# xxlong0/NeuralUDF

Measured on NVIDIA H100. Metric: ray-samples/sec (render_core fwd+bwd), higher is better.
Workload: dtype f32

## Files before the change

### neuraludf_b200/csrc/gemm_simt.cuh

```cuda
#pragma once
#include "common.cuh"

namespace nudf {

constexpr int GS_BM = 128, GS_BN = 128, GS_BK = 8, GS_PAD = 4, GS_THREADS = 256;

__device__ __forceinline__ unsigned long long pack2(float x, float y) {
  unsigned long long r;
  asm("mov.b64 %0, {%1, %2};" : "=l"(r) : "f"(x), "f"(y));
  return r;
}
__device__ __forceinline__ void unpack2(unsigned long long v, float& x, float& y) {
  asm("mov.b64 {%0, %1}, %2;" : "=f"(x), "=f"(y) : "l"(v));
}
__device__ __forceinline__ void ffma2(unsigned long long& d, unsigned long long a, unsigned long long b) {
  float dx, dy, ax, ay, bx, by;
  unpack2(d, dx, dy);
  unpack2(a, ax, ay);
  unpack2(b, bx, by);
  d = pack2(fmaf(ax, bx, dx), fmaf(ay, by, dy));
}

template <bool KC>
__device__ __forceinline__ float4 gs_fetch(const float* __restrict__ src, int64_t ld, int64_t mn0, int64_t mn_total, int k0,
// ... 125 lines not shown

__device__ __forceinline__ void ld4(const float* __restrict__ base, int64_t ld, int64_t row, int col, int nv, float out[4]) {
  const float* p = base + row * ld + col;
  if (nv == 4 && ((ld & 3) == 0) && ((col & 3) == 0) && aligned16(base)) {
    float4 t = *reinterpret_cast<const float4*>(p);
    out[0] = t.x; out[1] = t.y; out[2] = t.z; out[3] = t.w;
  } else {
#pragma unroll
    for (int j = 0; j < 4; ++j) out[j] = j < nv ? p[j] : 0.f;
  }
}
__device__ __forceinline__ void st4(float* __restrict__ base, int64_t ld, int64_t row, int col, int nv, const float v[4]) {
  float* p = base + row * ld + col;
  if (nv == 4 && ((ld & 3) == 0) && ((col & 3) == 0) && aligned16(base)) {
    *reinterpret_cast<float4*>(p) = make_float4(v[0], v[1], v[2], v[3]);
  } else {
#pragma unroll
    for (int j = 0; j < 4; ++j)
      if (j < nv) p[j] = v[j];
  }
}

#define NUDF_EPI_CALL                                                                                     \
  __device__ __forceinline__ void operator()(int64_t row, int col, const float acc[4], int nv) const {    \
    Aux aux;                                                                                              \
    load(row, col, nv, aux);                                                                              \
    apply(row, col, acc, nv, aux);                                                                        \
  }

struct EpiAct {
  float* C; int64_t ldc; const float* bias; int act; float post_scale;
  struct Aux { float b[4]; };
  __device__ __forceinline__ void load(int64_t, int col, int nv, Aux& x) const {
#pragma unroll
    for (int j = 0; j < 4; ++j) x.b[j] = (bias != nullptr && j < nv) ? bias[col + j] : 0.f;
  }
  __device__ __forceinline__ void apply(int64_t row, int col, const float acc[4], int nv, const Aux& x) const {
    float v[4];
#pragma unroll
    for (int j = 0; j < 4; ++j) {
      float t = acc[j] + x.b[j];
      if (act == ACT_RELU) t = fmaxf(t, 0.f);
      else if (act == ACT_SOFTPLUS100) t = softplus100(t);
      else if (act == ACT_SIGMOID) t = sigmoidf_(t);
      v[j] = t * post_scale;
    }
    st4(C, ldc, row, col, nv, v);
  }
  NUDF_EPI_CALL
};

struct EpiAtomicAdd {
  float* C; int64_t ldc;
  struct Aux {};
  __device__ __forceinline__ void load(int64_t, int, int, Aux&) const {}
  __device__ __forceinline__ void apply(int64_t row, int col, const float acc[4], int nv, const Aux&) const {
    float* p = C + row * ldc + col;
    if (nv == 4 && ((ldc & 3) == 0) && ((col & 3) == 0) && aligned16(C)) {
      asm volatile("red.global.add.v4.f32 [%0], {%1, %2, %3, %4};" ::"l"(p), "f"(acc[0]), "f"(acc[1]), "f"(acc[2]), "f"(acc[3])
                   : "memory");
      return;
    }
#pragma unroll
    for (int j = 0; j < 4; ++j)
      if (j < nv) atomicAdd(p + j, acc[j]);
  }
  NUDF_EPI_CALL
};


struct EpiSplitStore {
  float* ws; int64_t slice; int64_t ld;
  struct Aux {};
  __device__ __forceinline__ void load(int64_t, int, int, Aux&) const {}
  __device__ __forceinline__ void apply(int64_t row, int col, const float acc[4], int nv, const Aux&) const {
    float* p = ws + blockIdx.z * slice + row * ld + col;
#pragma unroll
    for (int j = 0; j < 4; ++j)
      if (j < nv) p[j] = acc[j];
  }
  NUDF_EPI_CALL
};

template <class Epi>
__global__ void splitk_reduce_kernel(const float* __restrict__ ws, int64_t slice, int splits, int64_t M, int N, Epi epi) {
  const int ncq = (N + 3) / 4;
  const int64_t idx = (int64_t)blockIdx.x * blockDim.x + threadIdx.x;
  const int64_t row = idx / ncq;
  if (row >= M) return;
  const int col = (int)(idx - row * ncq) * 4;
  const int nv = N - col < 4 ? N - col : 4;
  float x[4] = {0.f, 0.f, 0.f, 0.f};
  for (int z = 0; z < splits; ++z) {
    const float* p = ws + z * slice + row * N + col;
#pragma unroll
    for (int j = 0; j < 4; ++j)
      if (j < nv) x[j] += p[j];
  }
  epi(row, col, x, nv);
}
static __global__ void vec_reduce_kernel(const float* __restrict__ ws, int splits, int64_t n, float* __restrict__ out) {
  const int64_t i = (int64_t)blockIdx.x * blockDim.x + threadIdx.x;
  if (i >= n) return;
  float t = 0.f;
  for (int z = 0; z < splits; ++z) t += ws[z * n + i];
  out[i] += t;
}
template <class Epi>
static inline int splitk_reduce(const float* ws, int splits, int64_t M, int N, const Epi& epi, cudaStream_t st) {
  const int64_t n = M * ((N + 3) / 4);
  splitk_reduce_kernel<Epi><<<(unsigned)cdiv(n, 256), 256, 0, st>>>(ws, M * N, splits, M, N, epi);
  NUDF_LAUNCH_OK();
  return 0;
}
static inline int vec_reduce(const float* ws, int splits, int64_t n, float* out, cudaStream_t st) {
  vec_reduce_kernel<<<(unsigned)cdiv(n, 256), 256, 0, st>>>(ws, splits, n, out);
  NUDF_LAUNCH_OK();
  return 0;
}
static inline int ws_splits(int want, int64_t per_split) {
  const int64_t cap = SPLIT_WS_FLOATS / (per_split > 0 ? per_split : 1);
  return (int)(want < cap ? want : (cap < 1 ? 1 : cap));
}

struct EpiRev {
  int n_main; float post_scale;
  const float* Anext; int64_t lda; float a_unscale;
  float* Dprev; int64_t ldd;
  float* Gpe; int64_t ldg;
  struct Aux { float a[4]; };
  __device__ __forceinline__ void load(int64_t row, int col, int nv, Aux& x) const {
    int n = n_main - col;
    n = n < nv ? n : nv;
    if (n > 0) ld4(Anext, lda, row, col, n, x.a);
    else { x.a[0] = x.a[1] = x.a[2] = x.a[3] = 0.f; }
  }
  __device__ __forceinline__ void apply(int64_t row, int col, const float acc[4], int nv, const Aux& x) const {
    if (col + nv <= n_main) {
      float d[4];
#pragma unroll
      for (int j = 0; j < 4; ++j) d[j] = acc[j] * post_scale * sig_from_softplus(x.a[j] * a_unscale);
      st4(Dprev, ldd, row, col, nv, d);
      return;
    }
#pragma unroll
    for (int j = 0; j < 4; ++j) {
      if (j >= nv) break;
      int c = col + j;
      float g = acc[j] * post_scale;
      if (c < n_main) Dprev[row * ldd + c] = g * sig_from_softplus(x.a[j] * a_unscale);
      else if (Gpe != nullptr) Gpe[row * ldg + (c - n_main)] = g;
    }
  }
  NUDF_EPI_CALL
};

struct EpiRevFinal {
  float* Ge; int64_t ldge; const float* Gpe; int64_t ldg;
  struct Aux { float g[4]; };
  __device__ __forceinline__ void load(int64_t row, int col, int nv, Aux& x) const {
    if (Gpe != nullptr) ld4(Gpe, ldg, row, col, nv, x.g);
    else { x.g[0] = x.g[1] = x.g[2] = x.g[3] = 0.f; }
  }
  __device__ __forceinline__ void apply(int64_t row, int col, const float acc[4], int nv, const Aux& x) const {
    float v[4];
#pragma unroll
    for (int j = 0; j < 4; ++j) v[j] = acc[j] + x.g[j];
    st4(Ge, ldge, row, col, nv, v);
  }
  NUDF_EPI_CALL
};

struct EpiTan {
  const float* Anext; int64_t lda; float a_unscale;
  const float* D; int64_t ldd;
  float* Q; int64_t ldq;
  float* AdotNext; int64_t ldn; float post_scale;
  struct Aux { float a[4], d[4]; };
  __device__ __forceinline__ void load(int64_t row, int col, int nv, Aux& x) const {
    ld4(Anext, lda, row, col, nv, x.a);
    ld4(D, ldd, row, col, nv, x.d);
  }
  __device__ __forceinline__ void apply(int64_t row, int col, const float acc[4], int nv, const Aux& x) const {
    float q[4], n[4];
#pragma unroll
    for (int j = 0; j < 4; ++j) {
      float s = sig_from_softplus(x.a[j] * a_unscale);
      q[j] = acc[j] * x.d[j] * (100.0f * (1.0f - s));
      n[j] = s * acc[j] * post_scale;
    }
    st4(Q, ldq, row, col, nv, q);
    st4(AdotNext, ldn, row, col, nv, n);
  }
  NUDF_EPI_CALL
};

struct EpiBwd {
  int n_main; float post_scale;
  const float* Anext; int64_t lda; float a_unscale;
// ... 105 lines not shown
```

### neuraludf_b200/csrc/gemm_tc.cuh

```cuda
#pragma once
#include <cuda.h>
#include <cudaTypedefs.h>
#include <cuda_bf16.h>

#include "gemm_simt.cuh"

namespace nudf {
namespace tc {

constexpr int BM = 128;
constexpr int BN = 128;
constexpr int BK = 64;
constexpr int THREADS = 256;
constexpr int A_HALF_BYTES = BM * BK * 2;
__host__ __device__ constexpr int b_plane_bytes(int wn) { return wn * BK * 2; }
__host__ __device__ constexpr int acc_ld(int wn) { return wn + 4; }

__host__ __device__ inline int pad16(int n) { return (n + 15) & ~15; }
__host__ __device__ inline int pad64(int k) { return (k + 63) & ~63; }

__host__ __device__ inline uint32_t sw128(uint32_t row, uint32_t k) {
  return (row >> 3) * 1024u + (row & 7u) * 128u + ((((k >> 3) ^ (row & 7u)) & 7u) << 4) + ((k & 7u) << 1);
}

constexpr int TN_PS = 32;
constexpr int TN_RING = 4;
constexpr uint32_t TN_F32_OPND = TN_PS * BM * 4;
constexpr uint32_t TN_F32_STAGE = 2 * TN_F32_OPND;
constexpr uint32_t TN_PLANE = BM * TN_PS * 2;
constexpr uint32_t TN_PLANE_STAGE = 4 * TN_PLANE;
struct TnMaps { CUtensorMap a, b; };
__host__ __device__ inline uint32_t sw128_mn(uint32_t mn, uint32_t k) {
  return (mn >> 6) * 4096u + (k >> 3) * 1024u + (k & 7u) * 128u + ((((mn >> 3) ^ k) & 7u) << 4) + ((mn & 7u) << 1);
}

constexpr uint32_t W_SLOT = BM * BK * 4;
static_assert(W_SLOT == 2 * A_HALF_BYTES, "a slot holds exactly the two bf16 planes of its slice");
__host__ __device__ constexpr int w_ring(int wn) { return wn == 256 ? 3 : 4; }

__device__ __forceinline__ uint32_t pack_bf16(float a, float b) {
  __nv_bfloat162 v = __floats2bfloat162_rn(a, b);
  return *reinterpret_cast<uint32_t*>(&v);
}
template <int NP>
__device__ __forceinline__ void split4(const float x[4], uint2 planes[NP]) {
  float r[4] = {x[0], x[1], x[2], x[3]};
#pragma unroll
  for (int p = 0; p < NP; ++p) {
    const uint32_t a = pack_bf16(r[0], r[1]), b = pack_bf16(r[2], r[3]);
    planes[p] = make_uint2(a, b);
    r[0] -= __uint_as_float(a << 16);
    r[1] -= __uint_as_float(a & 0xffff0000u);
    r[2] -= __uint_as_float(b << 16);
    r[3] -= __uint_as_float(b & 0xffff0000u);
  }
}
__host__ __device__ inline int nt_of(int np) { return np == 2 ? 256 : 128; }
__host__ __device__ inline int n_tiles(int N, int np) { return (N + nt_of(np) - 1) / nt_of(np); }
__host__ __device__ inline int tile_rows(int N, int t, int np) { int r = N - nt_of(np) * t; return pad16(r < nt_of(np) ? r : nt_of(np)); }
__host__ __device__ inline int64_t tile_elems(int N, int K, int t, int np) { return (int64_t)(pad64(K) / 64) * np * tile_rows(N, t, np) * 64; }
__host__ __device__ inline int64_t tile_offset(int N, int K, int t, int np) {
  int64_t o = 0;
  for (int i = 0; i < t; ++i) o += tile_elems(N, K, i, np);
  return o;
}
__host__ __device__ inline int64_t image_elems(int N, int K, int np) { return tile_offset(N, K, n_tiles(N, np), np); }

static __device__ __forceinline__ void tc_prep_weights_body(const float* __restrict__ W, int64_t ldw, int N, int K, int transposed, int np,
                                                            uint16_t* __restrict__ img, int64_t start, int64_t stride) {
  const int Kp = pad64(K);
  const int nt = n_tiles(N, np);
  int64_t total = 0;
  for (int t = 0; t < nt; ++t) total += (int64_t)tile_rows(N, t, np) * Kp;
  for (int64_t idx = start; idx < total; idx += stride) {
    int64_t rem = idx;
    int t = 0;
    while (rem >= (int64_t)tile_rows(N, t, np) * Kp) { rem -= (int64_t)tile_rows(N, t, np) * Kp; ++t; }
    const int rows = tile_rows(N, t, np);
    const int nl = (int)(rem / Kp), k = (int)(rem - (int64_t)nl * Kp);
    const int n = t * nt_of(np) + nl;
    float x = 0.f;
    if (n < N && k < K) x = transposed ? W[(int64_t)k * ldw + n] : W[(int64_t)n * ldw + k];
    const int s = k >> 6, kl = k & 63;
    uint16_t* base = img + tile_offset(N, K, t, np) + (int64_t)s * np * rows * 64;
    const uint32_t off = sw128((uint32_t)nl, (uint32_t)kl) >> 1;
    float r = x;
    for (int p = 0; p < np; ++p) {
      __nv_bfloat16 h = __float2bfloat16_rn(r);
      base[(int64_t)p * rows * 64 + off] = __bfloat16_as_ushort(h);
      r -= __bfloat162float(h);
    }
  }
}
static __global__ void tc_prep_weights_kernel(const float* __restrict__ W, int64_t ldw, int N, int K, int transposed, int np,
                                              uint16_t* __restrict__ img) {
  tc_prep_weights_body(W, ldw, N, K, transposed, np, img, (int64_t)blockIdx.x * blockDim.x + threadIdx.x, (int64_t)gridDim.x * blockDim.x);
}


__device__ __forceinline__ uint32_t smem_u32(const void* p) { return (uint32_t)__cvta_generic_to_shared(p); }
__device__ __forceinline__ uint8_t* align1024(uint8_t* p) {
  return reinterpret_cast<uint8_t*>((reinterpret_cast<uintptr_t>(p) + 1023) & ~(uintptr_t)1023);
}

__device__ __forceinline__ void mbar_init(uint64_t* bar, uint32_t count) {
  asm volatile("mbarrier.init.shared::cta.b64 [%0], %1;" ::"r"(smem_u32(bar)), "r"(count) : "memory");
}
__device__ __forceinline__ void mbar_arrive(uint64_t* bar) {
  asm volatile("mbarrier.arrive.shared::cta.b64 _, [%0];" ::"r"(smem_u32(bar)) : "memory");
}
__device__ __forceinline__ void mbar_arrive_expect_tx(uint64_t* bar, uint32_t bytes) {
  asm volatile("mbarrier.arrive.expect_tx.shared::cta.b64 _, [%0], %1;" ::"r"(smem_u32(bar)), "r"(bytes) : "memory");
}
__device__ __forceinline__ uint32_t mbar_try_wait(uint32_t addr, uint32_t parity) {
  uint32_t ok;
  asm volatile(
      "{\n"
      ".reg .pred p;\n"
      "mbarrier.try_wait.parity.shared::cta.b64 p, [%1], %2;\n"
      "selp.u32 %0, 1, 0, p;\n"
      "}\n"
      : "=r"(ok)
      : "r"(addr), "r"(parity)
      : "memory");
  return ok;
}
__device__ __forceinline__ void mbar_wait(uint64_t* bar, uint32_t parity) {
  const uint32_t addr = smem_u32(bar);
  while (!mbar_try_wait(addr, parity)) {
  }
}
__device__ __forceinline__ void fence_barrier_init() { asm volatile("fence.mbarrier_init.release.cluster;" ::: "memory"); }
__device__ __forceinline__ void fence_proxy_async() { asm volatile("fence.proxy.async.shared::cta;" ::: "memory"); }

__device__ __forceinline__ void bulk_g2s(void* smem_dst, const void* gmem_src, uint32_t bytes, uint64_t* bar) {
  asm volatile("cp.async.bulk.shared::cluster.global.mbarrier::complete_tx::bytes [%0], [%1], %2, [%3];" ::"r"(smem_u32(smem_dst)),
               "l"(gmem_src), "r"(bytes), "r"(smem_u32(bar))
               : "memory");
}

__device__ __forceinline__ void tma_load_2d(void* smem_dst, const CUtensorMap* map, int c, int k, uint64_t* bar) {
  asm volatile("cp.async.bulk.tensor.2d.shared::cluster.global.mbarrier::complete_tx::bytes [%0], [%1, {%2, %3}], [%4];"
               ::"r"(smem_u32(smem_dst)), "l"(reinterpret_cast<uint64_t>(map)), "r"(c), "r"(k), "r"(smem_u32(bar))
               : "memory");
}

__device__ __forceinline__ uint64_t make_desc(uint32_t smem_addr) {
  return (uint64_t)((smem_addr & 0x3FFFFu) >> 4) | (1ull << 16) | (64ull << 32) | (1ull << 62);
}
__device__ __forceinline__ uint64_t make_desc_mn(uint32_t smem_addr) {
  return (uint64_t)((smem_addr & 0x3FFFFu) >> 4) | ((uint64_t)(4096 >> 4) << 16) | ((uint64_t)(1024 >> 4) << 32) | (1ull << 62);
}
__device__ __forceinline__ void wg_bar_sync() { asm volatile("bar.sync 1, 128;" ::: "memory"); }
template <uint32_t R> __device__ __forceinline__ void reg_dealloc() { asm volatile("setmaxnreg.dec.sync.aligned.u32 %0;" ::"n"(R)); }
template <uint32_t R> __device__ __forceinline__ void reg_alloc() { asm volatile("setmaxnreg.inc.sync.aligned.u32 %0;" ::"n"(R)); }
__device__ __forceinline__ void wg_fence() { asm volatile("wgmma.fence.sync.aligned;" ::: "memory"); }
__device__ __forceinline__ void wg_commit() { asm volatile("wgmma.commit_group.sync.aligned;" ::: "memory"); }
__device__ __forceinline__ void wg_wait_all() { asm volatile("wgmma.wait_group.sync.aligned 0;" ::: "memory"); }
__device__ __forceinline__ void wg_wait_but_one() { asm volatile("wgmma.wait_group.sync.aligned 1;" ::: "memory"); }
template <int N>
__device__ __forceinline__ void fence_operand(float (&d)[N]) {
#pragma unroll
  for (int q = 0; q < N; ++q) asm volatile("" : "+f"(d[q])::"memory");
}
__device__ __forceinline__ float unbias_rz(float r) { return fmaf(__uint_as_float(__float_as_uint(r) & 0xff800000u), 0x1p-24f, r); }

template <int MN_MAJOR = 0>
__device__ __forceinline__ void wgmma_128(float (&d)[64], uint64_t da, uint64_t db, uint32_t accumulate) {
  asm volatile(
      "{\n"
      ".reg .pred p;\n"
      "setp.ne.b32 p, %66, 0;\n"
      "wgmma.mma_async.sync.aligned.m64n128k16.f32.bf16.bf16 "
      "{%0, %1, %2, %3, %4, %5, %6, %7, %8, %9, %10, %11, %12, %13, %14, %15, %16, %17, %18, %19, %20, %21, %22, %23, %24, %25, "
      "%26, %27, %28, %29, %30, %31, %32, %33, %34, %35, %36, %37, %38, %39, %40, %41, %42, %43, %44, %45, %46, %47, %48, %49, "
      "%50, %51, %52, %53, %54, %55, %56, %57, %58, %59, %60, %61, %62, %63}, %64, %65, p, 1, 1, %67, %67;\n"
      "}\n"
      : "+f"(d[0]), "+f"(d[1]), "+f"(d[2]), "+f"(d[3]), "+f"(d[4]), "+f"(d[5]), "+f"(d[6]), "+f"(d[7]), "+f"(d[8]), "+f"(d[9]),
        "+f"(d[10]), "+f"(d[11]), "+f"(d[12]), "+f"(d[13]), "+f"(d[14]), "+f"(d[15]), "+f"(d[16]), "+f"(d[17]), "+f"(d[18]),
        "+f"(d[19]), "+f"(d[20]), "+f"(d[21]), "+f"(d[22]), "+f"(d[23]), "+f"(d[24]), "+f"(d[25]), "+f"(d[26]), "+f"(d[27]),
        "+f"(d[28]), "+f"(d[29]), "+f"(d[30]), "+f"(d[31]), "+f"(d[32]), "+f"(d[33]), "+f"(d[34]), "+f"(d[35]), "+f"(d[36]),
        "+f"(d[37]), "+f"(d[38]), "+f"(d[39]), "+f"(d[40]), "+f"(d[41]), "+f"(d[42]), "+f"(d[43]), "+f"(d[44]), "+f"(d[45]),
        "+f"(d[46]), "+f"(d[47]), "+f"(d[48]), "+f"(d[49]), "+f"(d[50]), "+f"(d[51]), "+f"(d[52]), "+f"(d[53]), "+f"(d[54]),
        "+f"(d[55]), "+f"(d[56]), "+f"(d[57]), "+f"(d[58]), "+f"(d[59]), "+f"(d[60]), "+f"(d[61]), "+f"(d[62]), "+f"(d[63])
      : "l"(da), "l"(db), "r"(accumulate), "n"(MN_MAJOR));
}
__device__ __forceinline__ void wgmma_128_fresh(float (&d)[64], uint64_t da, uint64_t db) {
  asm volatile(
      "{\n"
      ".reg .pred p;\n"
      "setp.ne.b32 p, %66, 0;\n"
      "wgmma.mma_async.sync.aligned.m64n128k16.f32.bf16.bf16 "
      "{%0, %1, %2, %3, %4, %5, %6, %7, %8, %9, %10, %11, %12, %13, %14, %15, %16, %17, %18, %19, %20, %21, %22, %23, %24, %25, "
      "%26, %27, %28, %29, %30, %31, %32, %33, %34, %35, %36, %37, %38, %39, %40, %41, %42, %43, %44, %45, %46, %47, %48, %49, "
      "%50, %51, %52, %53, %54, %55, %56, %57, %58, %59, %60, %61, %62, %63}, %64, %65, p, 1, 1, 0, 0;\n"
      "}\n"
      : "=f"(d[0]), "=f"(d[1]), "=f"(d[2]), "=f"(d[3]), "=f"(d[4]), "=f"(d[5]), "=f"(d[6]), "=f"(d[7]), "=f"(d[8]), "=f"(d[9]),
        "=f"(d[10]), "=f"(d[11]), "=f"(d[12]), "=f"(d[13]), "=f"(d[14]), "=f"(d[15]), "=f"(d[16]), "=f"(d[17]), "=f"(d[18]),
        "=f"(d[19]), "=f"(d[20]), "=f"(d[21]), "=f"(d[22]), "=f"(d[23]), "=f"(d[24]), "=f"(d[25]), "=f"(d[26]), "=f"(d[27]),
        "=f"(d[28]), "=f"(d[29]), "=f"(d[30]), "=f"(d[31]), "=f"(d[32]), "=f"(d[33]), "=f"(d[34]), "=f"(d[35]), "=f"(d[36]),
        "=f"(d[37]), "=f"(d[38]), "=f"(d[39]), "=f"(d[40]), "=f"(d[41]), "=f"(d[42]), "=f"(d[43]), "=f"(d[44]), "=f"(d[45]),
        "=f"(d[46]), "=f"(d[47]), "=f"(d[48]), "=f"(d[49]), "=f"(d[50]), "=f"(d[51]), "=f"(d[52]), "=f"(d[53]), "=f"(d[54]),
        "=f"(d[55]), "=f"(d[56]), "=f"(d[57]), "=f"(d[58]), "=f"(d[59]), "=f"(d[60]), "=f"(d[61]), "=f"(d[62]), "=f"(d[63])
      : "l"(da), "l"(db), "r"(0u));
}

__device__ __forceinline__ void wgmma_256(float (&d)[128], uint64_t da, uint64_t db, uint32_t accumulate) {
  asm volatile(
      "{\n"
      ".reg .pred p;\n"
      "setp.ne.b32 p, %130, 0;\n"
      "wgmma.mma_async.sync.aligned.m64n256k16.f32.bf16.bf16 "
      "{%0, %1, %2, %3, %4, %5, %6, %7, %8, %9, %10, %11, %12, %13, %14, %15, %16, %17, %18, %19, %20, %21, %22, %23, %24, "
      "%25, %26, %27, %28, %29, %30, %31, %32, %33, %34, %35, %36, %37, %38, %39, %40, %41, %42, %43, %44, %45, %46, %47, "
      "%48, %49, %50, %51, %52, %53, %54, %55, %56, %57, %58, %59, %60, %61, %62, %63, %64, %65, %66, %67, %68, %69, %70, "
      "%71, %72, %73, %74, %75, %76, %77, %78, %79, %80, %81, %82, %83, %84, %85, %86, %87, %88, %89, %90, %91, %92, %93, "
      "%94, %95, %96, %97, %98, %99, %100, %101, %102, %103, %104, %105, %106, %107, %108, %109, %110, %111, %112, %113, "
      "%114, %115, %116, %117, %118, %119, %120, %121, %122, %123, %124, %125, %126, %127}, %128, %129, p, 1, 1, 0, 0;\n"
      "}\n"
      : "+f"(d[0]), "+f"(d[1]), "+f"(d[2]), "+f"(d[3]), "+f"(d[4]), "+f"(d[5]), "+f"(d[6]), "+f"(d[7]), "+f"(d[8]),
        "+f"(d[9]), "+f"(d[10]), "+f"(d[11]), "+f"(d[12]), "+f"(d[13]), "+f"(d[14]), "+f"(d[15]), "+f"(d[16]), "+f"(d[17]),
        "+f"(d[18]), "+f"(d[19]), "+f"(d[20]), "+f"(d[21]), "+f"(d[22]), "+f"(d[23]), "+f"(d[24]), "+f"(d[25]), "+f"(d[26]),
        "+f"(d[27]), "+f"(d[28]), "+f"(d[29]), "+f"(d[30]), "+f"(d[31]), "+f"(d[32]), "+f"(d[33]), "+f"(d[34]), "+f"(d[35]),
        "+f"(d[36]), "+f"(d[37]), "+f"(d[38]), "+f"(d[39]), "+f"(d[40]), "+f"(d[41]), "+f"(d[42]), "+f"(d[43]), "+f"(d[44]),
        "+f"(d[45]), "+f"(d[46]), "+f"(d[47]), "+f"(d[48]), "+f"(d[49]), "+f"(d[50]), "+f"(d[51]), "+f"(d[52]), "+f"(d[53]),
        "+f"(d[54]), "+f"(d[55]), "+f"(d[56]), "+f"(d[57]), "+f"(d[58]), "+f"(d[59]), "+f"(d[60]), "+f"(d[61]), "+f"(d[62]),
        "+f"(d[63]), "+f"(d[64]), "+f"(d[65]), "+f"(d[66]), "+f"(d[67]), "+f"(d[68]), "+f"(d[69]), "+f"(d[70]), "+f"(d[71]),
        "+f"(d[72]), "+f"(d[73]), "+f"(d[74]), "+f"(d[75]), "+f"(d[76]), "+f"(d[77]), "+f"(d[78]), "+f"(d[79]), "+f"(d[80]),
        "+f"(d[81]), "+f"(d[82]), "+f"(d[83]), "+f"(d[84]), "+f"(d[85]), "+f"(d[86]), "+f"(d[87]), "+f"(d[88]), "+f"(d[89]),
        "+f"(d[90]), "+f"(d[91]), "+f"(d[92]), "+f"(d[93]), "+f"(d[94]), "+f"(d[95]), "+f"(d[96]), "+f"(d[97]), "+f"(d[98]),
        "+f"(d[99]), "+f"(d[100]), "+f"(d[101]), "+f"(d[102]), "+f"(d[103]), "+f"(d[104]), "+f"(d[105]), "+f"(d[106]),
        "+f"(d[107]), "+f"(d[108]), "+f"(d[109]), "+f"(d[110]), "+f"(d[111]), "+f"(d[112]), "+f"(d[113]), "+f"(d[114]),
        "+f"(d[115]), "+f"(d[116]), "+f"(d[117]), "+f"(d[118]), "+f"(d[119]), "+f"(d[120]), "+f"(d[121]), "+f"(d[122]),
        "+f"(d[123]), "+f"(d[124]), "+f"(d[125]), "+f"(d[126]), "+f"(d[127])
      : "l"(da), "l"(db), "r"(accumulate));
}
// ... 262 lines not shown
            const uint32_t off = sw128((uint32_t)(q * W3_QROWS + pass * 8 + rsub), (uint32_t)(c * 4));
#pragma unroll
            for (int p = 0; p < 3; ++p) *reinterpret_cast<uint2*>(st + p * A_HALF_BYTES + off) = pl[p];
          }
          fence_proxy_async();
          wg_bar_sync();
          if (tid == 0 && t1 < tiles) issue_quarter(t1, ks1, q);
        }
        fence_proxy_async();
        mbar_arrive(&full[s]);
      }
    }
  } else {
    reg_alloc<W3_CONSUMER_REGS>();
    const int cw = wg - 1, wtid = tid & 127, lane = tid & 31;
    float acc[64], acc2[64], tot[64];
    auto hi_hi = [&](float (&d)[64], uint32_t a, uint32_t b, int j) {
      wg_fence();
      wgmma_128_fresh(d, make_desc(a + 32u * j), make_desc(b + 32u * j));
      wg_commit();
    };
    auto add_unbiased = [&](float (&d)[64]) {
      fence_operand(d);
#pragma unroll
      for (int q = 0; q < 64; ++q) tot[q] += unbias_rz(d[q]);
    };
    uint32_t g = 0;
    for (int t = blockIdx.x; t < tiles; t += gridDim.x) {
      const int64_t m0 = (int64_t)(t / n_ct) * BM;
      const int n0 = (t % n_ct) * BN;
#pragma unroll
      for (int q = 0; q < 64; ++q) tot[q] = 0.f;
      for (int ks = 0; ks < n_slices; ++ks, ++g) {
        const int s = g & 1;
        mbar_wait(&full[s], (g >> 1) & 1);
        const uint32_t a = smem_u32(smem + s * W3_STAGE) + cw * (64 * 128), b = smem_u32(smem + s * W3_STAGE + W3_A_STAGE);
        wg_fence();
        mma_slice<3, BN>(acc, a, A_HALF_BYTES, b, B_PLANE, true);
        wg_commit();
        hi_hi(acc2, a, b, 0);
        wg_wait_but_one();
        fence_operand(acc);
#pragma unroll
        for (int q = 0; q < 64; ++q) tot[q] += acc[q];
        hi_hi(acc, a, b, 1);
        wg_wait_but_one();
        add_unbiased(acc2);
        hi_hi(acc2, a, b, 2);
        wg_wait_but_one();
        add_unbiased(acc);
        hi_hi(acc, a, b, 3);
        wg_wait_but_one();
        add_unbiased(acc2);
        wg_wait_all();
        mbar_arrive(&empty[s]);
        add_unbiased(acc);
      }
      const bool odd = lane & 1;
      const int64_t row = m0 + 64 * cw + 16 * (wtid >> 5) + (lane >> 2) + (odd ? 8 : 0);
      const int cbase = n0 + 4 * ((lane & 3) >> 1);
      constexpr int EPI_G = sizeof(typename Epi::Aux) <= 4 * sizeof(float) ? 8 : 4;
#pragma unroll
      for (int j0 = 0; j0 < 16; j0 += EPI_G) {
        typename Epi::Aux aux[EPI_G];
#pragma unroll
        for (int i = 0; i < EPI_G; ++i) {
          const int col = cbase + 8 * (j0 + i);
          if (row < M && col < N) epi.load(row, col, N - col < 4 ? N - col : 4, aux[i]);
        }
#pragma unroll
        for (int i = 0; i < EPI_G; ++i) {
          const int j = j0 + i, col = cbase + 8 * j;
          const float s0 = odd ? tot[4 * j] : tot[4 * j + 2], s1 = odd ? tot[4 * j + 1] : tot[4 * j + 3];
          const float r0 = __shfl_xor_sync(0xffffffffu, s0, 1), r1 = __shfl_xor_sync(0xffffffffu, s1, 1);
          const float x[4] = {odd ? r0 : tot[4 * j], odd ? r1 : tot[4 * j + 1], odd ? tot[4 * j + 2] : r0, odd ? tot[4 * j + 3] : r1};
          if (row < M && col < N) epi.apply(row, col, x, N - col < 4 ? N - col : 4, aux[i]);
        }
      }
    }
  }
}

template <class Epi>
__global__ void __launch_bounds__(THREADS, 1)
gemm_tn_kernel(int M, int N, int64_t K, int64_t k_chunk, Epi epi, float* __restrict__ colsum, float* __restrict__ cs_ws,
               const __grid_constant__ TnMaps maps) {
  extern __shared__ uint8_t smem_raw[];
  uint8_t* smem = align1024(smem_raw);
  const int tid = threadIdx.x, wg = tid >> 7, warp = tid >> 5, lane = tid & 31;
  const int m0 = blockIdx.x * BM;
  const int n0 = blockIdx.y * BN;
  const int64_t kb = (int64_t)blockIdx.z * k_chunk;
  const int64_t ke = (kb + k_chunk < K) ? kb + k_chunk : K;
  const bool do_csum = colsum != nullptr && blockIdx.y == 0;
  float csum[4] = {0.f, 0.f, 0.f, 0.f};
  if (ke <= kb) return;
  float acc[64];
#pragma unroll
  for (int q = 0; q < 64; ++q) acc[q] = 0.f;
  uint8_t* ring = smem;
  uint8_t* planes = smem + TN_RING * TN_F32_STAGE;
  float* cs_part = reinterpret_cast<float*>(planes + 2 * TN_PLANE_STAGE);
  uint64_t* full = reinterpret_cast<uint64_t*>(cs_part + 4 * BM);
  const int n_sl = (int)((ke - kb + TN_PS - 1) / TN_PS);
  const int opnd = warp >> 2, kq = warp & 3;

  auto issue = [&](int i) {
    const int r = i % TN_RING;
    const int k0 = (int)(kb + (int64_t)i * TN_PS);
    uint8_t* st = ring + r * TN_F32_STAGE;
    mbar_arrive_expect_tx(&full[r], TN_F32_STAGE);
    tma_load_2d(st, &maps.a, m0, k0, &full[r]);
    tma_load_2d(st + TN_F32_OPND, &maps.b, n0, k0, &full[r]);
  };
  auto split = [&](int i, uint8_t* dst) {
    const int r = i % TN_RING;
    mbar_wait(&full[r], (uint32_t)((i / TN_RING) & 1));
    const float* f = reinterpret_cast<const float*>(ring + r * TN_F32_STAGE + opnd * TN_F32_OPND) + 4 * lane;
    uint8_t* hi = dst + opnd * 2 * TN_PLANE;
    const int64_t k0 = kb + (int64_t)i * TN_PS;
#pragma unroll
    for (int q = 0; q < TN_PS / 8; ++q) {
      float4 v[2];
#pragma unroll
      for (int kk = 0; kk < 2; ++kk) {
        const int p = 8 * q + 2 * kq + kk;
        v[kk] = k0 + p < ke ? *reinterpret_cast<const float4*>(f + p * BM) : make_float4(0.f, 0.f, 0.f, 0.f);
      }
      if (opnd == 0 && do_csum) {
        csum[0] += v[0].x + v[1].x; csum[1] += v[0].y + v[1].y;
        csum[2] += v[0].z + v[1].z; csum[3] += v[0].w + v[1].w;
      }
#pragma unroll
      for (int kk = 0; kk < 2; ++kk) {
        const float x[4] = {v[kk].x, v[kk].y, v[kk].z, v[kk].w};
        uint2 pl[2];
        split4<2>(x, pl);
        const uint32_t off = sw128_mn(4u * lane, (uint32_t)(8 * q + 2 * kq + kk));
        *reinterpret_cast<uint2*>(hi + off) = pl[0];
        *reinterpret_cast<uint2*>(hi + TN_PLANE + off) = pl[1];
      }
    }
  };
  if (tid == 0) {
    for (int r = 0; r < TN_RING; ++r) mbar_init(&full[r], 1);
    fence_barrier_init();
    for (int i = 0; i < TN_RING && i < n_sl; ++i) issue(i);
  }
  __syncthreads();
  split(0, planes);
  fence_proxy_async();
  __syncthreads();
  if (tid == 0 && TN_RING < n_sl) issue(TN_RING);
  for (int i = 0; i < n_sl; ++i) {
    const int s = i & 1;
    const uint32_t st = smem_u32(planes + s * TN_PLANE_STAGE);
    wg_fence();
    mma_slice_mn(acc, st + wg * 4096u, st + 2 * TN_PLANE, i == 0);
    wg_commit();
    if (i + 1 < n_sl) split(i + 1, planes + (s ^ 1) * TN_PLANE_STAGE);
    wg_wait_all();
    fence_proxy_async();
    __syncthreads();
    if (tid == 0 && i + 1 + TN_RING < n_sl) issue(i + 1 + TN_RING);
  }
  if (do_csum && opnd == 0)
#pragma unroll
    for (int j = 0; j < 4; ++j) cs_part[kq * BM + 4 * lane + j] = csum[j];
  float* acc_s = reinterpret_cast<float*>(smem);
  acc_to_smem<BN>(acc, acc_s, wg, tid & 127);
  __syncthreads();
  if (do_csum && tid < BM && m0 + tid < M) {
    const float c = (cs_part[tid] + cs_part[BM + tid]) + (cs_part[2 * BM + tid] + cs_part[3 * BM + tid]);
    if (cs_ws != nullptr) cs_ws[(int64_t)blockIdx.z * M + m0 + tid] = c;
    else colsum[m0 + tid] += c;
  }
  tile_epilogue<BN>(acc_s, m0, M, n0, N, epi, tid);
}

static inline int sm_count() {
  static int n = 0;
  if (n == 0) {
    int dev = 0;
    if (cudaGetDevice(&dev) != cudaSuccess || cudaDeviceGetAttribute(&n, cudaDevAttrMultiProcessorCount, dev) != cudaSuccess || n <= 0) n = 132;
  }
  return n;
}


static inline int tensor_map_2d(CUtensorMap* map, const float* X, int64_t ld, int64_t cols, int64_t rows, int box_cols, int box_rows) {
  static PFN_cuTensorMapEncodeTiled encode = nullptr;
  if (encode == nullptr) {
    void* fn = nullptr;
    cudaDriverEntryPointQueryResult q;
    if (cudaGetDriverEntryPoint("cuTensorMapEncodeTiled", &fn, cudaEnableDefault, &q) != cudaSuccess || q != cudaDriverEntryPointSuccess ||
        fn == nullptr) {
      nudf::set_error("cuTensorMapEncodeTiled is not available from the driver");
      return -2;
    }
    encode = reinterpret_cast<PFN_cuTensorMapEncodeTiled>(fn);
  }
  const cuuint64_t dims[2] = {(cuuint64_t)cols, (cuuint64_t)rows};
  const cuuint64_t strides[1] = {(cuuint64_t)ld * sizeof(float)};
  const cuuint32_t box[2] = {(cuuint32_t)box_cols, (cuuint32_t)box_rows};
  const cuuint32_t elem[2] = {1, 1};
  const CUresult r = encode(map, CU_TENSOR_MAP_DATA_TYPE_FLOAT32, 2, const_cast<float*>(X), dims, strides, box, elem,
                            CU_TENSOR_MAP_INTERLEAVE_NONE, CU_TENSOR_MAP_SWIZZLE_NONE, CU_TENSOR_MAP_L2_PROMOTION_L2_256B,
                            CU_TENSOR_MAP_FLOAT_OOB_FILL_NONE);
  if (r != CUDA_SUCCESS) {
    nudf::set_error("cuTensorMapEncodeTiled failed (%d)", (int)r);
    return -2;
  }
  return 0;
}
static inline bool tma_operand_ok(const float* X, int64_t ld) { return (ld & 3) == 0 && aligned16(X); }
static inline int check_tma_operand(const float* X, int64_t ld) {
  if (tma_operand_ok(X, ld)) return 0;
  nudf::set_error("tensor-core operand at %p with row stride %lld floats: needs a stride of a multiple of 4 floats and a "
                  "16-byte-aligned base", (const void*)X, (long long)ld);
  return -1;
}

constexpr size_t w_ring_operand_bytes(int wn) { return (size_t)w_ring(wn) * W_SLOT + 2 * 2 * (size_t)b_plane_bytes(wn); }
constexpr size_t w_ring_smem_bytes(int wn) { return w_ring_operand_bytes(wn) + (w_ring(wn) + 2) * sizeof(uint64_t) + 1024; }
static_assert(w_ring_smem_bytes(BN) <= 227 * 1024 && w_ring_smem_bytes(2 * BN) <= 227 * 1024, "one CTA per SM");
static_assert(BM * acc_ld(BN) * sizeof(float) <= w_ring_operand_bytes(BN), "accumulator tile in the slots and stages");
static_assert(BM * acc_ld(2 * BN) * sizeof(float) <= w_ring_operand_bytes(2 * BN), "accumulator tile in the slots and stages");

template <int WN, class Epi>
static inline int gemm_w_launch(const float* A, int64_t lda, int64_t M, int N, int K, const uint16_t* img, const Epi& epi, cudaStream_t st) {
  constexpr size_t smem = w_ring_smem_bytes(WN);
  static bool attr_set = false;
  if (!attr_set) {
    NUDF_CUDA_OK(cudaFuncSetAttribute(gemm_w_kernel<WN, Epi>, cudaFuncAttributeMaxDynamicSharedMemorySize, (int)smem));
    attr_set = true;
  }
  CUtensorMap amap{};
  if (int rc = tensor_map_2d(&amap, A, lda, K > 0 ? K : 1, M, BK, BM)) return rc;
  const unsigned grid = (unsigned)(cdiv(M, BM) * cdiv(N, WN));
  LaunchTimer lt_(epi_family<Epi>::value, st);
  gemm_w_kernel<WN, Epi><<<grid, THREADS, smem, st>>>(M, N, K, img, epi, amap);
  NUDF_LAUNCH_OK();
  return 0;
}
constexpr size_t W3_SMEM = 2 * (size_t)W3_STAGE + W3_LAND + 8 * sizeof(uint64_t) + 1024;
static_assert(W3_SMEM <= 227 * 1024, "one CTA per SM");

template <class Epi>
static inline int gemm_w3_tma_launch(const float* A, int64_t lda, int64_t M, int N, int K, const uint16_t* img, const Epi& epi, cudaStream_t st) {
  static bool attr_set = false;
  if (!attr_set) {
    NUDF_CUDA_OK(cudaFuncSetAttribute(gemm_w3_tma_kernel<Epi>, cudaFuncAttributeMaxDynamicSharedMemorySize, (int)W3_SMEM));
    attr_set = true;
  }
  CUtensorMap amap{};
  if (int rc = tensor_map_2d(&amap, A, lda, K, M, BK, W3_QROWS)) return rc;
  const int64_t tiles = cdiv(M, BM) * cdiv(N, BN);
  const unsigned grid = (unsigned)(tiles < sm_count() ? tiles : sm_count());
  LaunchTimer lt_(epi_family<Epi>::value, st);
  gemm_w3_tma_kernel<Epi><<<grid, W3_THREADS, W3_SMEM, st>>>(A, M, N, K, img, epi, amap);
  NUDF_LAUNCH_OK();
  return 0;
}
template <int NP, class Epi>
static inline int gemm_w(const float* A, int64_t lda, int64_t M, int N, int K, const uint16_t* img, const Epi& epi, cudaStream_t st) {
  if (M <= 0 || N <= 0) return 0;
  if (int rc = check_tma_operand(A, lda)) return rc;
  if constexpr (NP == 3) {
    NUDF_REQUIRE(K > 0, "3-plane layers need K > 0");
    return gemm_w3_tma_launch<Epi>(A, lda, M, N, K, img, epi, st);
  } else {
    if (N > BN) return gemm_w_launch<2 * BN, Epi>(A, lda, M, N, K, img, epi, st);
    return gemm_w_launch<BN, Epi>(A, lda, M, N, K, img, epi, st);
  }
}

constexpr int TN_WAVE_CTAS = 132;
constexpr int64_t TN_MIN_POINTS = 512;
static inline int64_t tn_k_chunk(int M, int N, int64_t K) {
  const int64_t tiles = cdiv(M, BM) * cdiv(N, BN);
  int64_t splits = TN_WAVE_CTAS / tiles;
  if (splits > cdiv(K, TN_MIN_POINTS)) splits = cdiv(K, TN_MIN_POINTS);
  splits = ws_splits(splits < 1 ? 1 : (int)splits, (int64_t)M * N + M);
  return round_up(cdiv(K, splits), BK);
}

constexpr size_t TN_RING_SMEM = (size_t)TN_RING * TN_F32_STAGE + 2 * TN_PLANE_STAGE + 4 * BM * sizeof(float) + TN_RING * sizeof(uint64_t) + 1024;
static_assert(BM * acc_ld(BN) * sizeof(float) <= (size_t)TN_RING * TN_F32_STAGE, "accumulator tile in the ring");
static_assert(TN_RING_SMEM <= 227 * 1024, "one CTA per SM");

template <class Epi>
static inline int gemm_tn_launch(dim3 grid, const float* A, int64_t lda, const float* B, int64_t ldb, int M, int N, int64_t K,
                                 int64_t k_chunk, const Epi& epi, float* colsum, float* cs_ws, cudaStream_t st) {
  static bool attr_set = false;
  if (!attr_set) {
    NUDF_CUDA_OK(cudaFuncSetAttribute(gemm_tn_kernel<Epi>, cudaFuncAttributeMaxDynamicSharedMemorySize, (int)TN_RING_SMEM));
    attr_set = true;
  }
  TnMaps maps{};
  if (int rc = tensor_map_2d(&maps.a, A, lda, M, K, BM, TN_PS)) return rc;
  if (int rc = tensor_map_2d(&maps.b, B, ldb, N, K, BN, TN_PS)) return rc;
  gemm_tn_kernel<Epi><<<grid, THREADS, TN_RING_SMEM, st>>>(M, N, K, k_chunk, epi, colsum, cs_ws, maps);
  NUDF_LAUNCH_OK();
  return 0;
}
template <class Epi>
static inline int gemm_tn(const float* A, int64_t lda, const float* B, int64_t ldb, int M, int N, int64_t K, const Epi& epi,
                          cudaStream_t st, float* colsum_a = nullptr) {
  if (M <= 0 || N <= 0 || K <= 0) return 0;
  if (int rc = check_tma_operand(A, lda)) return rc;
  if (int rc = check_tma_operand(B, ldb)) return rc;
  const int64_t k_chunk = tn_k_chunk(M, N, K);
  const int splits = (int)cdiv(K, k_chunk);
  dim3 grid((unsigned)cdiv(M, BM), (unsigned)cdiv(N, BN), (unsigned)splits);
  LaunchTimer lt_(FAM_TC_WGRAD, st);
  if (splits == 1) return gemm_tn_launch(grid, A, lda, B, ldb, M, N, K, k_chunk, epi, colsum_a, nullptr, st);
  float* ws = split_workspace(st);
  if (ws == nullptr) return -2;
  float* cs = ws + (int64_t)splits * M * N;
  const EpiSplitStore e{ws, (int64_t)M * N, N};
  if (int rc = gemm_tn_launch(grid, A, lda, B, ldb, M, N, K, k_chunk, e, colsum_a, cs, st)) return rc;
  if (int rc = splitk_reduce(ws, splits, M, N, epi, st)) return rc;
  return colsum_a != nullptr ? vec_reduce(cs, splits, M, colsum_a, st) : 0;
}

struct PrepWJob { const float* W; uint16_t* img; int ldw, N, K, transposed, np; };
struct PrepWJobs { int n; PrepWJob j[64]; };
static __global__ void tc_prep_weights_jobs_kernel(const __grid_constant__ PrepWJobs jobs) {
  const PrepWJob& J = jobs.j[blockIdx.y];
  tc_prep_weights_body(J.W, J.ldw, J.N, J.K, J.transposed, J.np, J.img, (int64_t)blockIdx.x * blockDim.x + threadIdx.x,
                       (int64_t)gridDim.x * blockDim.x);
}
static inline int prep_weights_jobs(const PrepWJobs& jobs, cudaStream_t st) {
  if (jobs.n <= 0) return 0;
  int64_t mx = 0;
  for (int i = 0; i < jobs.n; ++i) {
    int64_t total = 0;
    for (int t = 0; t < n_tiles(jobs.j[i].N, jobs.j[i].np); ++t) total += (int64_t)tile_rows(jobs.j[i].N, t, jobs.j[i].np) * pad64(jobs.j[i].K);
    mx = total > mx ? total : mx;
  }
  int blocks = (int)((mx + 255) / 256);
  if (blocks > 1024) blocks = 1024;
  tc_prep_weights_jobs_kernel<<<dim3((unsigned)blocks, (unsigned)jobs.n), 256, 0, st>>>(jobs);
  NUDF_LAUNCH_OK();
  return 0;
}

static inline int prep_weights(const float* W, int64_t ldw, int N, int K, int transposed, int np, uint16_t* img, cudaStream_t st) {
  int64_t total = 0;
  for (int t = 0; t < n_tiles(N, np); ++t) total += (int64_t)tile_rows(N, t, np) * pad64(K);
  int blocks = (int)((total + 255) / 256);
  if (blocks > 4096) blocks = 4096;
  tc_prep_weights_kernel<<<blocks, 256, 0, st>>>(W, ldw, N, K, transposed, np, img);
  NUDF_LAUNCH_OK();
  return 0;
}

}
}
```

Measured before the change: 8.022 million.

## Warp-specialize weight-gradient TN GEMM and unroll split-K reductions

The weight-gradient TN GEMM becomes warp-specialized with 384 threads. One producer warpgroup converts the landed fp32 TMA slices into bf16 split planes across a 3-stage full/empty mbarrier ring, while two consumer warpgroups run wgmma with one group kept in flight and rebalanced registers via setmaxnreg. This is meant to overlap the fp32-to-bf16 split with the MMAs instead of serializing them behind block-wide syncs. Separately, the split-K reduce kernels gain 16-way unrolled float4 loads and smaller 64-thread blocks to expose more memory-level parallelism. The new design adds synchronization complexity and puts register pressure on the producer.

```diff
diff --git a/neuraludf_b200/csrc/gemm_simt.cuh b/neuraludf_b200/csrc/gemm_simt.cuh
--- a/neuraludf_b200/csrc/gemm_simt.cuh
+++ b/neuraludf_b200/csrc/gemm_simt.cuh
@@ -231,39 +231,63 @@
   NUDF_EPI_CALL
 };
 
+constexpr int SPLITK_UNROLL = 16, SPLITK_THREADS = 64;
+__device__ __forceinline__ float4 splitk_load4(const float* __restrict__ p, int nv, bool vec) {
+  if (vec) return __ldg(reinterpret_cast<const float4*>(p));
+  float4 r = make_float4(0.f, 0.f, 0.f, 0.f);
+  if (nv > 0) r.x = __ldg(p);
+  if (nv > 1) r.y = __ldg(p + 1);
+  if (nv > 2) r.z = __ldg(p + 2);
+  if (nv > 3) r.w = __ldg(p + 3);
+  return r;
+}
 template <class Epi>
-__global__ void splitk_reduce_kernel(const float* __restrict__ ws, int64_t slice, int splits, int64_t M, int N, Epi epi) {
+__global__ void __launch_bounds__(SPLITK_THREADS) splitk_reduce_kernel(const float* __restrict__ ws, int64_t slice, int splits, int64_t M, int N, Epi epi) {
   const int ncq = (N + 3) / 4;
   const int64_t idx = (int64_t)blockIdx.x * blockDim.x + threadIdx.x;
   const int64_t row = idx / ncq;
   if (row >= M) return;
   const int col = (int)(idx - row * ncq) * 4;
   const int nv = N - col < 4 ? N - col : 4;
+  const float* p = ws + row * N + col;
+  const bool vec = nv == 4 && (N & 3) == 0 && (slice & 3) == 0 && aligned16(ws);
   float x[4] = {0.f, 0.f, 0.f, 0.f};
-  for (int z = 0; z < splits; ++z) {
-    const float* p = ws + z * slice + row * N + col;
-#pragma unroll
-    for (int j = 0; j < 4; ++j)
-      if (j < nv) x[j] += p[j];
-  }
+  auto add = [&](const float4& v) { x[0] += v.x; x[1] += v.y; x[2] += v.z; x[3] += v.w; };
+  int z = 0;
+  for (; z + SPLITK_UNROLL <= splits; z += SPLITK_UNROLL) {
+    float4 v[SPLITK_UNROLL];
+#pragma unroll
+    for (int u = 0; u < SPLITK_UNROLL; ++u) v[u] = splitk_load4(p + (z + u) * slice, nv, vec);
+#pragma unroll
+    for (int u = 0; u < SPLITK_UNROLL; ++u) add(v[u]);
+  }
+  for (; z < splits; ++z) add(splitk_load4(p + z * slice, nv, vec));
   epi(row, col, x, nv);
 }
-static __global__ void vec_reduce_kernel(const float* __restrict__ ws, int splits, int64_t n, float* __restrict__ out) {
+static __global__ void __launch_bounds__(SPLITK_THREADS) vec_reduce_kernel(const float* __restrict__ ws, int splits, int64_t n, float* __restrict__ out) {
   const int64_t i = (int64_t)blockIdx.x * blockDim.x + threadIdx.x;
   if (i >= n) return;
   float t = 0.f;
-  for (int z = 0; z < splits; ++z) t += ws[z * n + i];
+  int z = 0;
+  for (; z + SPLITK_UNROLL <= splits; z += SPLITK_UNROLL) {
+    float v[SPLITK_UNROLL];
+#pragma unroll
+    for (int u = 0; u < SPLITK_UNROLL; ++u) v[u] = __ldg(ws + (z + u) * n + i);
+#pragma unroll
+    for (int u = 0; u < SPLITK_UNROLL; ++u) t += v[u];
+  }
+  for (; z < splits; ++z) t += ws[z * n + i];
   out[i] += t;
 }
 template <class Epi>
 static inline int splitk_reduce(const float* ws, int splits, int64_t M, int N, const Epi& epi, cudaStream_t st) {
   const int64_t n = M * ((N + 3) / 4);
-  splitk_reduce_kernel<Epi><<<(unsigned)cdiv(n, 256), 256, 0, st>>>(ws, M * N, splits, M, N, epi);
+  splitk_reduce_kernel<Epi><<<(unsigned)cdiv(n, SPLITK_THREADS), SPLITK_THREADS, 0, st>>>(ws, M * N, splits, M, N, epi);
   NUDF_LAUNCH_OK();
   return 0;
 }
 static inline int vec_reduce(const float* ws, int splits, int64_t n, float* out, cudaStream_t st) {
-  vec_reduce_kernel<<<(unsigned)cdiv(n, 256), 256, 0, st>>>(ws, splits, n, out);
+  vec_reduce_kernel<<<(unsigned)cdiv(n, SPLITK_THREADS), SPLITK_THREADS, 0, st>>>(ws, splits, n, out);
   NUDF_LAUNCH_OK();
   return 0;
 }
diff --git a/neuraludf_b200/csrc/gemm_tc.cuh b/neuraludf_b200/csrc/gemm_tc.cuh
--- a/neuraludf_b200/csrc/gemm_tc.cuh
+++ b/neuraludf_b200/csrc/gemm_tc.cuh
@@ -24,7 +24,11 @@
 }
 
 constexpr int TN_PS = 32;
-constexpr int TN_RING = 4;
+constexpr int TN_LAND = 4;
+constexpr int TN_STAGES = 3;
+constexpr int TN_THREADS = 384;
+constexpr int TN_PRODUCER_REGS = 104, TN_CONSUMER_REGS = 200;
+static_assert(TN_PRODUCER_REGS + 2 * TN_CONSUMER_REGS <= 65536 / 128, "register file of one SM");
 constexpr uint32_t TN_F32_OPND = TN_PS * BM * 4;
 constexpr uint32_t TN_F32_STAGE = 2 * TN_F32_OPND;
 constexpr uint32_t TN_PLANE = BM * TN_PS * 2;
@@ -99,9 +103,7 @@
 
 
 __device__ __forceinline__ uint32_t smem_u32(const void* p) { return (uint32_t)__cvta_generic_to_shared(p); }
-__device__ __forceinline__ uint8_t* align1024(uint8_t* p) {
-  return reinterpret_cast<uint8_t*>((reinterpret_cast<uintptr_t>(p) + 1023) & ~(uintptr_t)1023);
-}
+__device__ __forceinline__ uint8_t* align1024(uint8_t* p) { return p + ((1024u - (smem_u32(p) & 1023u)) & 1023u); }
 
 __device__ __forceinline__ void mbar_init(uint64_t* bar, uint32_t count) {
   asm volatile("mbarrier.init.shared::cta.b64 [%0], %1;" ::"r"(smem_u32(bar)), "r"(count) : "memory");
@@ -152,6 +154,7 @@
   return (uint64_t)((smem_addr & 0x3FFFFu) >> 4) | ((uint64_t)(4096 >> 4) << 16) | ((uint64_t)(1024 >> 4) << 32) | (1ull << 62);
 }
 __device__ __forceinline__ void wg_bar_sync() { asm volatile("bar.sync 1, 128;" ::: "memory"); }
+__device__ __forceinline__ void tn_consumer_bar_sync() { asm volatile("bar.sync 2, 256;" ::: "memory"); }
 template <uint32_t R> __device__ __forceinline__ void reg_dealloc() { asm volatile("setmaxnreg.dec.sync.aligned.u32 %0;" ::"n"(R)); }
 template <uint32_t R> __device__ __forceinline__ void reg_alloc() { asm volatile("setmaxnreg.inc.sync.aligned.u32 %0;" ::"n"(R)); }
 __device__ __forceinline__ void wg_fence() { asm volatile("wgmma.fence.sync.aligned;" ::: "memory"); }
@@ -580,100 +583,124 @@
 }
 
 template <class Epi>
-__global__ void __launch_bounds__(THREADS, 1)
+__global__ void __launch_bounds__(TN_THREADS, 1)
 gemm_tn_kernel(int M, int N, int64_t K, int64_t k_chunk, Epi epi, float* __restrict__ colsum, float* __restrict__ cs_ws,
                const __grid_constant__ TnMaps maps) {
   extern __shared__ uint8_t smem_raw[];
   uint8_t* smem = align1024(smem_raw);
-  const int tid = threadIdx.x, wg = tid >> 7, warp = tid >> 5, lane = tid & 31;
+  const int tid = threadIdx.x, wg = tid >> 7, lane = tid & 31;
   const int m0 = blockIdx.x * BM;
   const int n0 = blockIdx.y * BN;
   const int64_t kb = (int64_t)blockIdx.z * k_chunk;
   const int64_t ke = (kb + k_chunk < K) ? kb + k_chunk : K;
   const bool do_csum = colsum != nullptr && blockIdx.y == 0;
-  float csum[4] = {0.f, 0.f, 0.f, 0.f};
   if (ke <= kb) return;
-  float acc[64];
-#pragma unroll
-  for (int q = 0; q < 64; ++q) acc[q] = 0.f;
-  uint8_t* ring = smem;
-  uint8_t* planes = smem + TN_RING * TN_F32_STAGE;
-  float* cs_part = reinterpret_cast<float*>(planes + 2 * TN_PLANE_STAGE);
-  uint64_t* full = reinterpret_cast<uint64_t*>(cs_part + 4 * BM);
+  uint8_t* land = smem;
+  uint8_t* planes = smem + TN_LAND * TN_F32_STAGE;
+  float* acc_s = reinterpret_cast<float*>(land);
+  float* cs_part = acc_s + BM * acc_ld(BN);
+  uint64_t* landed = reinterpret_cast<uint64_t*>(planes + TN_STAGES * TN_PLANE_STAGE);
+  uint64_t* full = landed + TN_LAND;
+  uint64_t* empty = full + TN_STAGES;
   const int n_sl = (int)((ke - kb + TN_PS - 1) / TN_PS);
-  const int opnd = warp >> 2, kq = warp & 3;
 
   auto issue = [&](int i) {
-    const int r = i % TN_RING;
+    const int r = i % TN_LAND;
     const int k0 = (int)(kb + (int64_t)i * TN_PS);
-    uint8_t* st = ring + r * TN_F32_STAGE;
-    mbar_arrive_expect_tx(&full[r], TN_F32_STAGE);
-    tma_load_2d(st, &maps.a, m0, k0, &full[r]);
-    tma_load_2d(st + TN_F32_OPND, &maps.b, n0, k0, &full[r]);
-  };
-  auto split = [&](int i, uint8_t* dst) {
-    const int r = i % TN_RING;
-    mbar_wait(&full[r], (uint32_t)((i / TN_RING) & 1));
-    const float* f = reinterpret_cast<const float*>(ring + r * TN_F32_STAGE + opnd * TN_F32_OPND) + 4 * lane;
-    uint8_t* hi = dst + opnd * 2 * TN_PLANE;
-    const int64_t k0 = kb + (int64_t)i * TN_PS;
-#pragma unroll
-    for (int q = 0; q < TN_PS / 8; ++q) {
-      float4 v[2];
-#pragma unroll
-      for (int kk = 0; kk < 2; ++kk) {
-        const int p = 8 * q + 2 * kq + kk;
-        v[kk] = k0 + p < ke ? *reinterpret_cast<const float4*>(f + p * BM) : make_float4(0.f, 0.f, 0.f, 0.f);
-      }
-      if (opnd == 0 && do_csum) {
-        csum[0] += v[0].x + v[1].x; csum[1] += v[0].y + v[1].y;
-        csum[2] += v[0].z + v[1].z; csum[3] += v[0].w + v[1].w;
-      }
-#pragma unroll
-      for (int kk = 0; kk < 2; ++kk) {
-        const float x[4] = {v[kk].x, v[kk].y, v[kk].z, v[kk].w};
-        uint2 pl[2];
-        split4<2>(x, pl);
-        const uint32_t off = sw128_mn(4u * lane, (uint32_t)(8 * q + 2 * kq + kk));
-        *reinterpret_cast<uint2*>(hi + off) = pl[0];
-        *reinterpret_cast<uint2*>(hi + TN_PLANE + off) = pl[1];
-      }
-    }
+    uint8_t* st = land + r * TN_F32_STAGE;
+    mbar_arrive_expect_tx(&landed[r], TN_F32_STAGE);
+    tma_load_2d(st, &maps.a, m0, k0, &landed[r]);
+    tma_load_2d(st + TN_F32_OPND, &maps.b, n0, k0, &landed[r]);
   };
   if (tid == 0) {
-    for (int r = 0; r < TN_RING; ++r) mbar_init(&full[r], 1);
+    for (int r = 0; r < TN_LAND; ++r) mbar_init(&landed[r], 1);
+    for (int s = 0; s < TN_STAGES; ++s) {
+      mbar_init(&full[s], 128);
+      mbar_init(&empty[s], 256);
+    }
     fence_barrier_init();
-    for (int i = 0; i < TN_RING && i < n_sl; ++i) issue(i);
+    for (int i = 0; i < TN_LAND && i < n_sl; ++i) issue(i);
   }
   __syncthreads();
-  split(0, planes);
-  fence_proxy_async();
-  __syncthreads();
-  if (tid == 0 && TN_RING < n_sl) issue(TN_RING);
-  for (int i = 0; i < n_sl; ++i) {
-    const int s = i & 1;
-    const uint32_t st = smem_u32(planes + s * TN_PLANE_STAGE);
-    wg_fence();
-    mma_slice_mn(acc, st + wg * 4096u, st + 2 * TN_PLANE, i == 0);
-    wg_commit();
-    if (i + 1 < n_sl) split(i + 1, planes + (s ^ 1) * TN_PLANE_STAGE);
+
+  if (wg == 0) {
+    reg_dealloc<TN_PRODUCER_REGS>();
+    const int kq = tid >> 5;
+    float csum[4] = {0.f, 0.f, 0.f, 0.f};
+    for (int i = 0; i < n_sl; ++i) {
+      const int r = i % TN_LAND, s = i % TN_STAGES;
+      uint8_t* st = planes + s * TN_PLANE_STAGE;
+      mbar_wait(&empty[s], ((i / TN_STAGES) & 1) ^ 1);
+      mbar_wait(&landed[r], (i / TN_LAND) & 1);
+      const int64_t left = ke - (kb + (int64_t)i * TN_PS);
+      const int np = left < TN_PS ? (int)left : TN_PS;
+      const float* f = reinterpret_cast<const float*>(land + r * TN_F32_STAGE) + 4 * lane;
+      float4 v[2][TN_PS / 8][2];
+#pragma unroll
+      for (int opnd = 0; opnd < 2; ++opnd)
+#pragma unroll
+        for (int q = 0; q < TN_PS / 8; ++q)
+#pragma unroll
+          for (int kk = 0; kk < 2; ++kk) {
+            const int p = 8 * q + 2 * kq + kk;
+            v[opnd][q][kk] = p < np ? *reinterpret_cast<const float4*>(f + opnd * (TN_F32_OPND / 4) + p * BM) : make_float4(0.f, 0.f, 0.f, 0.f);
+          }
+      if (do_csum)
+#pragma unroll
+        for (int q = 0; q < TN_PS / 8; ++q) {
+          csum[0] += v[0][q][0].x + v[0][q][1].x; csum[1] += v[0][q][0].y + v[0][q][1].y;
+          csum[2] += v[0][q][0].z + v[0][q][1].z; csum[3] += v[0][q][0].w + v[0][q][1].w;
+        }
+#pragma unroll
+      for (int opnd = 0; opnd < 2; ++opnd)
+#pragma unroll
+        for (int q = 0; q < TN_PS / 8; ++q)
+#pragma unroll
+          for (int kk = 0; kk < 2; ++kk) {
+            const float x[4] = {v[opnd][q][kk].x, v[opnd][q][kk].y, v[opnd][q][kk].z, v[opnd][q][kk].w};
+            uint2 pl[2];
+            split4<2>(x, pl);
+            const uint32_t off = sw128_mn(4u * lane, (uint32_t)(8 * q + 2 * kq + kk));
+            *reinterpret_cast<uint2*>(st + opnd * 2 * TN_PLANE + off) = pl[0];
+            *reinterpret_cast<uint2*>(st + opnd * 2 * TN_PLANE + TN_PLANE + off) = pl[1];
+          }
+      fence_proxy_async();
+      mbar_arrive(&full[s]);
+      wg_bar_sync();
+      if (tid == 0 && i + TN_LAND < n_sl) issue(i + TN_LAND);
+    }
+    if (do_csum)
+#pragma unroll
+      for (int j = 0; j < 4; ++j) cs_part[kq * BM + 4 * lane + j] = csum[j];
+    __syncthreads();
+    if (do_csum && m0 + tid < M) {
+      const float c = (cs_part[tid] + cs_part[BM + tid]) + (cs_part[2 * BM + tid] + cs_part[3 * BM + tid]);
+      if (cs_ws != nullptr) cs_ws[(int64_t)blockIdx.z * M + m0 + tid] = c;
+      else colsum[m0 + tid] += c;
+    }
+  } else {
+    reg_alloc<TN_CONSUMER_REGS>();
+    const int cw = wg - 1;
+    float acc[64];
+#pragma unroll
+    for (int q = 0; q < 64; ++q) acc[q] = 0.f;
+    for (int i = 0; i < n_sl; ++i) {
+      const int s = i % TN_STAGES;
+      mbar_wait(&full[s], (i / TN_STAGES) & 1);
+      const uint32_t st = smem_u32(planes + s * TN_PLANE_STAGE);
+      wg_fence();
+      mma_slice_mn(acc, st + cw * 4096u, st + 2 * TN_PLANE, i == 0);
+      wg_commit();
+      wg_wait_but_one();
+      if (i > 0) mbar_arrive(&empty[(i - 1) % TN_STAGES]);
+    }
     wg_wait_all();
-    fence_proxy_async();
+    fence_operand(acc);
     __syncthreads();
-    if (tid == 0 && i + 1 + TN_RING < n_sl) issue(i + 1 + TN_RING);
-  }
-  if (do_csum && opnd == 0)
-#pragma unroll
-    for (int j = 0; j < 4; ++j) cs_part[kq * BM + 4 * lane + j] = csum[j];
-  float* acc_s = reinterpret_cast<float*>(smem);
-  acc_to_smem<BN>(acc, acc_s, wg, tid & 127);
-  __syncthreads();
-  if (do_csum && tid < BM && m0 + tid < M) {
-    const float c = (cs_part[tid] + cs_part[BM + tid]) + (cs_part[2 * BM + tid] + cs_part[3 * BM + tid]);
-    if (cs_ws != nullptr) cs_ws[(int64_t)blockIdx.z * M + m0 + tid] = c;
-    else colsum[m0 + tid] += c;
-  }
-  tile_epilogue<BN>(acc_s, m0, M, n0, N, epi, tid);
+    acc_to_smem<BN>(acc, acc_s, cw, tid & 127);
+    tn_consumer_bar_sync();
+    tile_epilogue<BN>(acc_s, m0, M, n0, N, epi, tid - 128);
+  }
 }
 
 static inline int sm_count() {
@@ -783,22 +810,23 @@
   return round_up(cdiv(K, splits), BK);
 }
 
-constexpr size_t TN_RING_SMEM = (size_t)TN_RING * TN_F32_STAGE + 2 * TN_PLANE_STAGE + 4 * BM * sizeof(float) + TN_RING * sizeof(uint64_t) + 1024;
-static_assert(BM * acc_ld(BN) * sizeof(float) <= (size_t)TN_RING * TN_F32_STAGE, "accumulator tile in the ring");
-static_assert(TN_RING_SMEM <= 227 * 1024, "one CTA per SM");
+constexpr size_t TN_SMEM = (size_t)TN_LAND * TN_F32_STAGE + (size_t)TN_STAGES * TN_PLANE_STAGE +
+                           (TN_LAND + 2 * TN_STAGES) * sizeof(uint64_t) + 1024;
+static_assert((BM * acc_ld(BN) + 4 * BM) * sizeof(float) <= (size_t)TN_LAND * TN_F32_STAGE, "accumulator tile and column sums in the landing ring");
+static_assert(TN_SMEM <= 227 * 1024, "one CTA per SM");
 
 template <class Epi>
 static inline int gemm_tn_launch(dim3 grid, const float* A, int64_t lda, const float* B, int64_t ldb, int M, int N, int64_t K,
                                  int64_t k_chunk, const Epi& epi, float* colsum, float* cs_ws, cudaStream_t st) {
   static bool attr_set = false;
   if (!attr_set) {
-    NUDF_CUDA_OK(cudaFuncSetAttribute(gemm_tn_kernel<Epi>, cudaFuncAttributeMaxDynamicSharedMemorySize, (int)TN_RING_SMEM));
+    NUDF_CUDA_OK(cudaFuncSetAttribute(gemm_tn_kernel<Epi>, cudaFuncAttributeMaxDynamicSharedMemorySize, (int)TN_SMEM));
     attr_set = true;
   }
   TnMaps maps{};
   if (int rc = tensor_map_2d(&maps.a, A, lda, M, K, BM, TN_PS)) return rc;
   if (int rc = tensor_map_2d(&maps.b, B, ldb, N, K, BN, TN_PS)) return rc;
-  gemm_tn_kernel<Epi><<<grid, THREADS, TN_RING_SMEM, st>>>(M, N, K, k_chunk, epi, colsum, cs_ws, maps);
+  gemm_tn_kernel<Epi><<<grid, TN_THREADS, TN_SMEM, st>>>(M, N, K, k_chunk, epi, colsum, cs_ws, maps);
   NUDF_LAUNCH_OK();
   return 0;
 }
```

Result: faster. 8.270 million, median of 6 (+3.1%).
